# lab-incert/peba1

Hardware: AMD Instinct MI355X
Metric: bootstrapped gates/sec (blind rotations/s) over the PEBA1 match path, and end-to-end match ms (higher is better)
Workload: dtype u32

## Files before the change

### __graft_entry__.py

```python
import os
import subprocess
import sys
import tempfile

ROOT = os.path.dirname(os.path.abspath(__file__))
if ROOT not in sys.path:
    sys.path.insert(0, ROOT)


def build():
    from peba1_amd.kernel_id import kernels_sha16
    mix_path = os.path.join(ROOT, "profiles", "isa_mix.json")
    sha, stale = kernels_sha16(), True
    if os.path.exists(mix_path):
        import json
        with open(mix_path) as f:
            stale = json.load(f).get("kernels_sha16") != sha
    env = dict(os.environ)
    asm = os.path.join(tempfile.gettempdir(), f"peba1_kernels_{sha}.s")
    if stale:
        env["EMIT_KERNEL_ASM"] = asm
    subprocess.check_call(["bash", os.path.join(ROOT, "peba1_amd", "csrc", "build.sh")], env=env)
    if stale:
        try:
            subprocess.check_call([sys.executable, os.path.join(ROOT, "tools", "isa_mix.py"), asm, "--json", mix_path, "--sha", sha],
                                  stdout=subprocess.DEVNULL)
        except (subprocess.CalledProcessError, OSError) as e:
            print(f"__graft_entry__.build: tools/isa_mix.py could not summarise the kernel listing ({e}); "
                  f"profiles/isa_mix.json left as it was", file=sys.stderr)
        if os.path.exists(asm):
            os.remove(asm)
    subprocess.check_call(["make", "-s", "-C", os.path.join(ROOT, "oracle")])
    if os.path.exists("/root/reference/src/Math.cpp"):
        subprocess.check_call(["make", "-s", "-C", os.path.join(ROOT, "oracle"), "ref"])
    import peba1_amd
    from peba1_amd import lib, circuits, dist
    lib.load()
    circuits.load()
    dist.load()


def smoke():
    import numpy as np
    from oracle import pyoracle as O
    from peba1_amd import api, lib

    L = lib.load()
    seed = 0x5EBA2
    pp = api.ParameterSet(128)
    ks = api.SecretKeySet(pp, seed, device=True)
    oks = O.KeySet(O.params("P128"), seed)
    L.tfhe_hip_set_encrypt_seed(1)
    a = api.CiphertextArray(pp, 4).encrypt([0, 0, 1, 1], ks)
    b = api.CiphertextArray(pp, 4).encrypt([0, 1, 0, 1], ks)
# ... 19 lines not shown
```

### include/tfhe_hip.h

```cpp
#ifndef TFHE_HIP_H
#define TFHE_HIP_H

#include <stdio.h>

#include "tfhe/tfhe_core.h"

#ifdef __cplusplus
extern "C" {
#endif

enum TfheHipGate {
    TFHE_HIP_NAND = 0, TFHE_HIP_OR, TFHE_HIP_AND, TFHE_HIP_NOR, TFHE_HIP_XOR, TFHE_HIP_XNOR,
    TFHE_HIP_ANDNY, TFHE_HIP_ANDYN, TFHE_HIP_ORNY, TFHE_HIP_ORYN
};

const char *tfhe_hip_last_error(void);
void tfhe_hip_clear_error(void);

int tfhe_hip_set_device(int device);
int tfhe_hip_get_device(void);
int tfhe_hip_device_pci_bus_id(char *out, int len);

TFheGateBootstrappingParameterSet *tfhe_hip_new_parameters(
    int32_t n, int32_t N, int32_t k, int32_t l, int32_t Bgbit, int32_t ks_t, int32_t ks_basebit,
// ... 150 lines not shown

int tfhe_hip_test_stage_place(int64_t pos, int64_t capacity, int32_t outstanding, int64_t bytes, int64_t *out4);

void tfhe_hip_test_set_alloc_cap(int64_t bytes);

int tfhe_hip_test_schedule(const int32_t *ops5, int32_t count, int32_t unit, int32_t balance, int32_t *levels_out);
int tfhe_hip_test_level_plan(const int32_t *ops5, const int32_t *op_keys, int32_t count, int32_t nkeys, int32_t unit,
                             int32_t balance, int32_t *levels_out, int32_t *sizes6, int32_t *rot_off, int32_t *ks_off,
                             int32_t *rot_koff, int32_t *ks_koff, int32_t *rot_key, int32_t *rots6, int32_t *kss4);
int tfhe_hip_test_level_plan3(const int32_t *ops5, const int32_t *op_keys, int32_t count, int32_t nkeys, int32_t unit,
                              int32_t balance, int32_t *levels_out, int32_t *sizes6, int32_t *rot_off, int32_t *ks_off,
                              int32_t *rot_koff, int32_t *ks_koff, int32_t *rot_key, int32_t *rots8, int32_t *kss4);
int tfhe_hip_test_level_plan_lut(const int32_t *ops10, const int32_t *op_keys, int32_t count, int32_t nkeys, int32_t unit,
                                 int32_t balance, int32_t reuse, int32_t *levels_out, int32_t *shared_with, int32_t *sizes6,
                                 int32_t *rot_off, int32_t *ks_off, int32_t *rot_koff, int32_t *ks_koff, int32_t *rot_key,
                                 int32_t *rots9, int32_t *kss4);
int tfhe_hip_test_level_plan_multi(const int32_t *ops16, const int32_t *op_keys, int32_t count, int32_t nkeys, int32_t unit,
                                   int32_t balance, int32_t reuse, const int32_t *dead_slots, int32_t ndead,
                                   int32_t *levels_out, int32_t *shared_with, int32_t *sizes6, int32_t *rot_off, int32_t *ks_off,
                                   int32_t *rot_koff, int32_t *ks_koff, int32_t *rot_key, int32_t *rots10, int32_t *kss4);
int tfhe_hip_test_level_plan_lin(const int32_t *ops16, const int32_t *op_keys, int32_t count, int32_t nkeys, int32_t unit,
                                 int32_t balance, int32_t reuse, const int32_t *dead_slots, int32_t ndead,
                                 const int32_t *lin_terms2, int32_t nterms, int32_t *levels_out, int32_t *ranks_out,
                                 int32_t *shared_with, int32_t *sizes6, int32_t *rot_off, int32_t *ks_off, int32_t *rot_koff,
                                 int32_t *ks_koff, int32_t *rot_key, int32_t *rots10, int32_t *kss4, int32_t *lin_sizes2,
                                 int32_t *lin_level_off, int32_t *lin_launch_off, int32_t *lin_launch_rank, int32_t *lins35);
int tfhe_hip_test_level_plan_full(const int32_t *ops16, const int32_t *op_keys, int32_t count, int32_t nkeys, int32_t unit,
                                  int32_t balance, int32_t reuse, const int32_t *dead_slots, int32_t ndead,
                                  const int32_t *lin_terms2, int32_t nterms, int32_t *levels_out, int32_t *ranks_out,
                                  int32_t *shared_with, int32_t *sizes6, int32_t *rot_off, int32_t *ks_off, int32_t *rot_koff,
                                  int32_t *ks_koff, int32_t *rot_key, int32_t *rots10, int32_t *kss4, int32_t *lin_sizes2,
                                  int32_t *lin_level_off, int32_t *lin_launch_off, int32_t *lin_launch_rank, int32_t *lins35,
                                  int32_t *not_off, int32_t *nots2);
int tfhe_hip_test_br_plan(int32_t N, int32_t l, int32_t Bgbit, const int32_t *tunings4, int32_t cu_count, int32_t count,
                          int32_t flags, int32_t *out3);
int tfhe_hip_test_ks_plan(int32_t n, int32_t N, int32_t k, int32_t ks_t, int32_t ks_basebit, const int32_t *tunings5,
                          int32_t cu_count, int32_t count, int64_t *out6);
int tfhe_hip_test_ks_plan_form(int32_t n, int32_t N, int32_t k, int32_t ks_t, int32_t ks_basebit, const int32_t *tunings5,
                               int32_t cu_count, int32_t count, int64_t *out7);
int tfhe_hip_test_wg_times(const TFheGateBootstrappingCloudKeySet *bk, int32_t width, uint64_t *times4, double *launch_ms);

typedef struct TfheHipPackingKey TfheHipPackingKey;
TfheHipPackingKey *tfhe_hip_new_packing_key(const TFheGateBootstrappingSecretKeySet *secret, int32_t pk_t, int32_t pk_basebit);
TfheHipPackingKey *tfhe_hip_new_packing_key_seeded(const TFheGateBootstrappingSecretKeySet *secret, int32_t pk_t,
                                                   int32_t pk_basebit, uint64_t seed);
TfheHipPackingKey *tfhe_hip_new_packing_key_from_words(const TFheGateBootstrappingParameterSet *params, int32_t pk_t,
                                                       int32_t pk_basebit, const Torus32 *words);
void tfhe_hip_delete_packing_key(TfheHipPackingKey *key);
const Torus32 *tfhe_hip_packing_key_words(const TfheHipPackingKey *key, int64_t *count);
int tfhe_hip_packing_key_decomposition(const TfheHipPackingKey *key, int32_t *pk_t, int32_t *pk_basebit);
int tfhe_hip_pack_samples(const TfheHipPackingKey *key, const LweSample *samples, int32_t count,
                          const TFheGateBootstrappingCloudKeySet *bk, Torus32 *out_words);
int tfhe_hip_pack_samples_device(const TfheHipPackingKey *key, const LweSample *samples, int32_t count,
                                 const TFheGateBootstrappingCloudKeySet *bk, void *device_words);
int tfhe_hip_packed_phase(const TFheGateBootstrappingSecretKeySet *secret, const Torus32 *words, Torus32 *out_phases);
int tfhe_hip_packed_decrypt_bits(const TFheGateBootstrappingSecretKeySet *secret, const Torus32 *words, int32_t count,
                                 int32_t *out_bits);
int tfhe_hip_test_pack_bounds(int32_t N, int32_t rows, int32_t basebit);

int tfhe_hip_ring_encrypt(const TFheGateBootstrappingSecretKeySet *secret, const Torus32 *mu, Torus32 *out_words);
int tfhe_hip_ring_encrypt_seeded(const TFheGateBootstrappingSecretKeySet *secret, const Torus32 *mu, Torus32 *out_words,
                                 uint64_t seed);
int tfhe_hip_ring_encrypt_bits(const TFheGateBootstrappingSecretKeySet *secret, const int32_t *bits, int32_t count,
                               Torus32 *out_words);
int tfhe_hip_ring_encrypt_bits_seeded(const TFheGateBootstrappingSecretKeySet *secret, const int32_t *bits, int32_t count,
                                      Torus32 *out_words, uint64_t seed);
// ... 129 lines not shown
```

### peba1_amd/csrc/launch_plan.hpp

```cpp
#pragma once
#include <algorithm>
#include <cstddef>

#include "br_forms.hpp"

namespace tfhe_hip {

struct LaunchTunings {
    int br_variant = -1;
    int br8_max_rotations = 1 << 30;
    int br_tail8 = 1;
    int br_digit_table = 1;
    int ks_target_blocks = 32768;
    int ks_max_splits = 48;
    int ks_split_ties = 0;
    int ks_tile = 16;
    int ks_index = 1;
};

inline void fill_form_ok(bool form_ok[BR_FORM_COUNT][3], int N, int l, int Bgbit) {
    for (int f = 0; f < BR_FORM_COUNT; ++f)
        for (int t = 0; t < 3; ++t) form_ok[f][t] = br_form_admissible(f, N, l, Bgbit, t);
}

struct BrPlan { int form; int tables; int tail; };

inline BrPlan plan_br(const bool form_ok[BR_FORM_COUNT][3], int N, int l, const LaunchTunings &t, int cu_count, int count,
                      bool stamps, bool acc_dump) {
    int form;
    if (t.br_variant == 4 && N == 1024) form = BR_FORM_WAVE2;
    else if (t.br_variant == 2 || N == 2048) form = BR_FORM_SPLIT;
    else if (t.br8_max_rotations > 0 && count <= std::min(t.br8_max_rotations, cu_count) && l >= 2 && !stamps)
        form = BR_FORM_WAVE8;
    else form = BR_FORM_WIDE4;
    if (stamps && N == 1024) form = BR_FORM_WIDE4;
// ... 34 lines not shown
                       (threads == 128 || threads == 192 || threads == 320);
    if (!tiled) return KsPlan{KS_FORM_PERGATE, 0};
    return KsPlan{t.ks_index ? KS_FORM_INDEX : KS_FORM_STRIP, tile};
}

inline bool ks_tiled(const LaunchTunings &t, int count, const KsShape &p) { return plan_ks(t, count, p).form != KS_FORM_PERGATE; }

inline int ks_splits(const LaunchTunings &t, int cu_count, int cnt, const KsShape &p) {
    int splits = 1;
    const KsPlan plan = plan_ks(t, cnt, p);
    if (plan.form != KS_FORM_PERGATE) {
        const int tile = plan.tile;
        const int threads = ks_threads(p);
        int per_cu = std::max(1, (tile == 16 ? 16 : tile == 24 ? 12 : 8) / (threads / 64));
        if (plan.form == KS_FORM_STRIP) {
            const size_t lds = (size_t)16 * threads * 16 + (size_t)tile * 65 * 4;
            per_cu = std::max(1, std::min((int)((160 * 1024) / lds), 8 / (threads / 64)));
        }
        const long long slots = (long long)cu_count * per_cu;
        const long long tiles = (cnt + tile - 1) / tile;
        const int lo = std::max(2, (p.nin + 63) / 64);
        double best = -1.0;
        for (int sp = lo; sp <= t.ks_max_splits; ++sp) {
            const long long blocks = tiles * sp, rounds = (blocks + slots - 1) / slots;
            const double eff = (double)blocks / (double)(rounds * slots);
            if (t.ks_split_ties ? eff >= best - 1e-9 : eff > best + 1e-9) { best = eff; splits = sp; }
        }
    } else {
        while (splits < t.ks_max_splits && cnt * splits * 2 <= t.ks_target_blocks) splits *= 2;
    }
    return splits;
}

inline size_t ks_partial_bytes(const LaunchTunings &t, int cu_count, int count, const KsShape &p) {
    size_t most = 0;
    const int chunk = ks_tiled(t, count, p) ? KS_CHUNK : count;
    for (int done = 0; done < count; done += chunk) {
        const int cnt = std::min(chunk, count - done), splits = ks_splits(t, cu_count, cnt, p);
        if (splits > 1) most = std::max(most, (size_t)cnt * splits * p.ct_stride * 4);
    }
    return most;
}

}
```

### peba1_amd/csrc/recorder.cpp

```cpp
#include "recorder.hpp"

#include <algorithm>
#include <cstdio>
#include <cstdlib>
#include <cstring>
#include <utility>
#include <vector>

#include "op_graph.hpp"

namespace tfhe_hip {
namespace {

const uint8_t GATE_TT[10][4] = {
    {1, 1, 1, 0}, {0, 1, 1, 1}, {0, 0, 0, 1}, {1, 0, 0, 0}, {0, 1, 1, 0}, {1, 0, 0, 1},
    {0, 1, 0, 0}, {0, 0, 1, 0}, {1, 1, 0, 1}, {1, 0, 1, 1},
};

struct Recorder {
    std::recursive_mutex mtx;
    bool deferred = true;
    std::vector<const TFheGateBootstrappingCloudKeySet *> keys;
    uint16_t cur_key = 0;
    SlotPool *pool = nullptr;
    bool batch_keys = false;
    OpGraph<SlotPool> graph;
    bool balance_levels = true;
    std::vector<PendingOp> flight_ops;
    std::vector<LinTerm> flight_terms;
    SlotPool *flight_pool = nullptr;
    std::vector<const TFheGateBootstrappingCloudKeySet *> flight_keys;
    bool eliminate_dead = true;
    bool fold_constants = false;
};
Recorder &rec() {
    static Recorder r;
    static bool init = [] {
        if (const char *e = std::getenv("TFHE_HIP_DEFERRED")) r.deferred = std::atoi(e) != 0;
        if (const char *e = std::getenv("TFHE_HIP_FOLD_CONSTANTS")) r.fold_constants = std::atoi(e) != 0;
        if (const char *e = std::getenv("TFHE_HIP_BATCH_KEYS")) r.batch_keys = std::atoi(e) != 0;
        return true;
    }();
    (void)init;
    return r;
}

void release_refs(SlotPool *pool, const PendingOp &op, const LinTerm *terms) {
    for_each_src(op, terms, [&](int32_t s) { pool->release(s); });
    for_each_dst(op, [&](int32_t d) { pool->release(d); });
}

bool same_evaluation_params(const Params &a, const Params &b) {
    return a.n == b.n && a.N == b.N && a.k == b.k && a.l == b.l && a.Bgbit == b.Bgbit && a.ks_t == b.ks_t &&
           a.ks_basebit == b.ks_basebit;
}

void select_key(const TFheGateBootstrappingCloudKeySet *bk) {
    Recorder &r = rec();
    auto known = std::find(r.keys.begin(), r.keys.end(), bk);
    if (known == r.keys.end() && !r.graph.ops().empty()) {
        if (!r.batch_keys || pool_of_key(bk) != r.pool || !same_evaluation_params(bk->bk->p, r.keys.front()->bk->p))
            flush_locked();
    }
    if (r.graph.ops().empty()) r.keys.clear();
    known = std::find(r.keys.begin(), r.keys.end(), bk);
    if (known == r.keys.end()) {
        if (r.keys.size() > UINT16_MAX) flush_locked();
        if (r.graph.ops().empty()) r.keys.clear();
        r.keys.push_back(bk);
        known = r.keys.end() - 1;
    }
    r.cur_key = (uint16_t)(known - r.keys.begin());
}
// ... 253 lines not shown
        std::memset(result->a, 0, (size_t)bk->params->in_out_params->n * sizeof(Torus32));
        result->b = value ? (1 << 29) : -(1 << 29);
    }
}

void record_copy_locked(LweSample *result, const LweSample *ca, const TFheGateBootstrappingCloudKeySet *bk) {
    Recorder &r = rec();
    begin_op(bk);
    if (result == ca) return;
    bind_pool(result, r.pool);
    const int32_t s = ensure_slot(ca, r.pool);
    r.pool->retain(s);
    repoint(result, r.pool, s);
    if (!r.deferred) sync_sample_locked(result);
}

void finish_flight_locked() {
    Recorder &r = rec();
    Engine::get().wait_flight();
    for (const PendingOp &op : r.flight_ops) release_refs(r.flight_pool, op, r.flight_terms.data());
    r.flight_ops.clear();
    r.flight_terms.clear();
    r.flight_pool = nullptr;
    r.flight_keys.clear();
}

int flush_locked(bool wait) {
    Recorder &r = rec();
    if (!r.graph.ops().empty() && r.eliminate_dead) Engine::get().stats.dead_gates += r.graph.eliminate_dead(*r.pool);
    if (r.graph.ops().empty()) { if (wait) finish_flight_locked(); return 0; }
    SlotPool *pool = r.pool;
    const std::vector<PendingOp> &ops = r.graph.ops();
    std::vector<int32_t> lvl, alap;
    const int levels = schedule_levels(ops, r.graph.max_level(), r.balance_levels, Engine::get().cu_count(), lvl, &alap, r.graph.terms());
    if (const char *trace = std::getenv("TFHE_HIP_TRACE_DAG")) {
        if (FILE *f = std::fopen(trace, "w")) {
            for (size_t i = 0; i < ops.size(); ++i)
                std::fprintf(f, "%d %d %d %d %d %d %d %d\n", (int)ops[i].kind, ops[i].level, alap[i], lvl[i],
                             ops[i].dst, ops[i].a, ops[i].b, ops[i].c);
            std::fclose(f);
        }
    }
    std::vector<int32_t> remap(r.keys.size(), -1);
    for (const PendingOp &op : ops) remap[op.key] = 0;
    std::vector<const TFheGateBootstrappingCloudKeySet *> used;
    std::vector<const DeviceKeyImage *> images;
    for (size_t k = 0; k < r.keys.size(); ++k)
        if (remap[k] == 0) { remap[k] = (int32_t)used.size(); used.push_back(r.keys[k]); images.push_back(r.keys[k]->bk->dev); }
    LevelPlan plan;
    if (used.size() == r.keys.size()) {
        plan = build_level_plan(ops, lvl, levels, (int)used.size(), r.graph.terms());
    } else {
        std::vector<PendingOp> rekeyed = ops;
        for (PendingOp &op : rekeyed) op.key = (uint16_t)remap[op.key];
        plan = build_level_plan(rekeyed, lvl, levels, (int)used.size(), r.graph.terms());
    }
    finish_flight_locked();
    Engine::get().execute(images, pool, std::move(plan), wait);
    for (const PendingOp &op : ops) {
        for_each_dst(op, [&](int32_t d) {
            pool->level[d] = 0;
            pool->pending[d] = 0;
        });
        if (wait) release_refs(pool, op, r.graph.terms());
    }
    if (!wait) { r.flight_pool = pool; r.flight_keys = std::move(used); }
    r.graph.clear(wait ? nullptr : &r.flight_ops, wait ? nullptr : &r.flight_terms);
    return levels;
}

void flush_pending_locked(bool wait) { if (!rec().graph.ops().empty()) flush_locked(wait); }

void forget_key_locked(const TFheGateBootstrappingCloudKeySet *bk) {
    Recorder &r = rec();
    const bool pending = std::find(r.keys.begin(), r.keys.end(), bk) != r.keys.end();
    const bool flying = std::find(r.flight_keys.begin(), r.flight_keys.end(), bk) != r.flight_keys.end();
    if (pending || flying) { flush_locked(); r.keys.clear(); }
}

bool deferred_mode() { return rec().deferred; }

bool set_deferred_locked(bool on) { return std::exchange(rec().deferred, on); }

bool set_batch_keys_locked(bool on) { return std::exchange(rec().batch_keys, on); }

bool set_recorder_tuning_locked(const char *name, bool on) {
    Recorder &r = rec();
    bool *knob = std::strcmp(name, "reuse_gates") == 0      ? &r.graph.reuse
                 : std::strcmp(name, "eliminate_dead") == 0 ? &r.eliminate_dead
                 : std::strcmp(name, "fold_constants") == 0 ? &r.fold_constants
                 : std::strcmp(name, "balance_levels") == 0 ? &r.balance_levels
                 : std::strcmp(name, "batch_keys") == 0     ? &r.batch_keys
                                                            : nullptr;
    if (knob) *knob = on;
    return knob != nullptr;
}

}
```

### peba1_amd/csrc/recorder.hpp

```cpp
#pragma once
#include <cstdint>
#include <mutex>

#include "engine.hpp"
#include "../../include/tfhe/tfhe.h"

namespace tfhe_hip {
#pragma GCC visibility push(hidden)

constexpr int32_t SLOT_HOST = -1;
constexpr int32_t SLOT_ZERO = -2;

void bind_pool(const LweSample *sample, SlotPool *pool);
SlotPool *pool_of_sample(const LweSample *sample);

std::unique_lock<std::recursive_mutex> recorder_lock();
SlotPool *pool_of_key(const TFheGateBootstrappingCloudKeySet *bk);

void record_gate2_locked(int code, LweSample *result, const LweSample *a, const LweSample *b,
                         const TFheGateBootstrappingCloudKeySet *bk);
void record_not_locked(LweSample *result, const LweSample *a, const TFheGateBootstrappingCloudKeySet *bk);
void record_mux_locked(LweSample *result, const LweSample *a, const LweSample *b, const LweSample *c,
                       const TFheGateBootstrappingCloudKeySet *bk);
void record_gate3_locked(int gate, int negate_mask, LweSample *result, const LweSample *a, const LweSample *b,
                         const LweSample *c, const TFheGateBootstrappingCloudKeySet *bk);
void record_lut_locked(int32_t lut, LweSample *result, int nin, const LweSample *const *in, const int32_t *coef, int32_t c0,
                       const TFheGateBootstrappingCloudKeySet *bk);
void record_lutm_locked(int32_t lut, int32_t spec, int nout, LweSample *const *result, int nin, const LweSample *const *in,
                        const int32_t *coef, int32_t c0, const TFheGateBootstrappingCloudKeySet *bk);
void record_linear_locked(LweSample *result, int nin, const LweSample *const *in, const int32_t *coef, int32_t c0,
                          const TFheGateBootstrappingCloudKeySet *bk);
void forget_lutm_locked(int32_t lut, int32_t spec);
void forget_lut_locked(int32_t lut);
void record_constant_locked(LweSample *result, int32_t value, const TFheGateBootstrappingCloudKeySet *bk);
void record_copy_locked(LweSample *result, const LweSample *a, const TFheGateBootstrappingCloudKeySet *bk);

int32_t alloc_slot(SlotPool *pool);
int32_t ensure_slot(const LweSample *s, SlotPool *pool);
void repoint(LweSample *s, SlotPool *pool, int32_t slot);
void sync_sample_locked(const LweSample *s);

int flush_locked(bool wait = true);
void flush_pending_locked(bool wait = true);
void finish_flight_locked();
void forget_key_locked(const TFheGateBootstrappingCloudKeySet *bk);
bool deferred_mode();
bool set_deferred_locked(bool on);
bool set_batch_keys_locked(bool on);
bool set_recorder_tuning_locked(const char *name, bool on);
#pragma GCC visibility pop

}
```

### peba1_amd/csrc/scheduler.cpp

```cpp
#include "scheduler.hpp"

#include "engine.hpp"

#include <algorithm>
#include <queue>
#include <unordered_map>

namespace tfhe_hip {

namespace {
struct HeapItem {
    int32_t alap, idx;
    bool operator>(const HeapItem &o) const { return alap != o.alap ? alap > o.alap : idx > o.idx; }
};
}


int schedule_levels(const std::vector<PendingOp> &ops, int asap_depth, bool balance, int unit,
                    std::vector<int32_t> &lvl, std::vector<int32_t> *alap_out, const LinTerm *terms) {
    const int n = (int)ops.size();
    lvl.resize(n);
    for (int i = 0; i < n; ++i) lvl[i] = ops[i].level;
    if (alap_out) *alap_out = lvl;
    if (!balance || asap_depth <= 2 || n < 4 * unit) return asap_depth;

    int32_t max_slot = -1;
    for (int i = 0; i < n; ++i) for_each_dst(ops[i], [&](int32_t d) { max_slot = std::max(max_slot, d); });
    std::vector<int32_t> producer((size_t)max_slot + 1, -1);
    for (int i = 0; i < n; ++i)
        for_each_dst(ops[i], [&](int32_t d) { if (producer[d] < 0) producer[d] = i; });

    std::vector<size_t> pred_at(n);
    size_t pred_room = 0;
    for (int i = 0; i < n; ++i) { pred_at[i] = pred_room; pred_room += 3 + (size_t)op_terms(ops[i]); }
    std::vector<int32_t> pred(pred_room, -1), npred(n, 0), succ_off(n + 1, 0);
    for (int i = 0; i < n; ++i) {
        for_each_src(ops[i], terms, [&](int32_t src) {
            const int32_t pr = src <= max_slot ? producer[src] : -1;
            if (pr < 0 || pr >= i) return;
            bool dup = false;
            for (int t = 0; t < npred[i]; ++t) dup |= pred[pred_at[i] + t] == pr;
            if (dup) return;
            pred[pred_at[i] + npred[i]++] = pr;
            ++succ_off[pr + 1];
        });
    }
    for (int i = 0; i < n; ++i) succ_off[i + 1] += succ_off[i];
    std::vector<int32_t> succ(succ_off[n]), cursor(succ_off.begin(), succ_off.end() - 1);
    for (int i = 0; i < n; ++i)
        for (int t = 0; t < npred[i]; ++t) succ[cursor[pred[pred_at[i] + t]]++] = i;

    std::vector<int32_t> alap(n, asap_depth);
// ... 42 lines not shown
    std::vector<int32_t> batch;
    std::vector<long long> due(asap_depth + 2, 0);
    for (int i = 0; i < n; ++i) due[alap[i]] += op_rotations(ops[i]);
    for (int L = 1; L <= asap_depth; ++L) {
        for (int32_t i : avail[L]) heap.push(HeapItem{alap[i], i});
        const long long levels_left = asap_depth - L + 1;
        const long long base = remaining <= (long long)unit * levels_left ? unit : 2LL * unit;
        long long cap = base, running = 0, excess = 0;
        const int horizon = std::min(asap_depth, L + 1023);
        for (int D = L; D <= horizon; ++D) {
            running += due[D];
            excess = std::max(excess, running - base * (long long)(D - L + 1));
        }
        while (excess > cap - base && cap < 16LL * unit) cap *= 2;
        long long width = 0;
        batch.clear();
        auto take = [&](long long limit, bool forced_only) {
            while (!heap.empty()) {
                const HeapItem top = heap.top();
                const int w = op_rotations(ops[top.idx]);
                if (top.alap > L && (forced_only || width + w > limit)) break;
                heap.pop();
                lvl[top.idx] = L;
                width += w;
                due[top.alap] -= w;
                batch.push_back(top.idx);
            }
        };
        take(cap, false);
        if (width > cap) take((width + 2LL * unit - 1) / (2LL * unit) * (2LL * unit), false);
        remaining -= width;
        for (int32_t i : batch) release_successors(i, L, release_successors);
    }
    return asap_depth;
}

static void plan_linear_ops(LevelPlan &plan, const std::vector<PendingOp> &ops, const std::vector<int32_t> &lvl, int levels,
                            const LinTerm *terms) {
    int32_t max_slot = -1;
    size_t nlin = 0;
    for (const PendingOp &op : ops)
        if (op.kind == OP_LIN) { max_slot = std::max(max_slot, op.dst); ++nlin; }
    if (!nlin) return;
    std::vector<int32_t> producer((size_t)max_slot + 1, -1);
    plan.op_rank.assign(ops.size(), 0);
    std::vector<std::pair<int64_t, int32_t>> order;
    order.reserve(nlin);
    for (size_t i = 0; i < ops.size(); ++i) {
        const PendingOp &op = ops[i];
        if (op.kind != OP_LIN) continue;
        int32_t rank = 0;
        for (int t = 0; t < op.nout; ++t) {
            const int32_t s = terms[op.spec + t].slot;
            const int32_t pr = s <= max_slot ? producer[(size_t)s] : -1;
            if (pr >= 0 && lvl[(size_t)pr] == lvl[i]) rank = std::max(rank, plan.op_rank[(size_t)pr] + 1);
        }
        plan.op_rank[i] = rank;
        producer[(size_t)op.dst] = (int32_t)i;
        order.emplace_back((int64_t)lvl[i] << 32 | (uint32_t)rank, (int32_t)i);
    }
    std::stable_sort(order.begin(), order.end(), [](const auto &x, const auto &y) { return x.first < y.first; });
    plan.lins.resize(nlin);
    plan.lin_level_off.assign((size_t)levels + 2, 0);
    plan.lin_launch_off.assign(1, 0);
    for (size_t j = 0; j < nlin; ++j) {
        const PendingOp &op = ops[(size_t)order[j].second];
// ... 103 lines not shown
```

### peba1_amd/csrc/scheduler.hpp

```cpp
#pragma once
#include <cstddef>
#include <cstdint>
#include <utility>
#include <vector>

namespace tfhe_hip {

struct PendingOp {
    uint8_t kind;
    int32_t dst, a, b, c;
    int32_t level;
    uint16_t key = 0;
    int32_t lut = -1;
    int32_t sa = 0, sb = 0, sc = 0, c0 = 0;
    int32_t spec = -1;
    int32_t nout = 0;
    int32_t dsts[4] = {-1, -1, -1, -1};
};
constexpr uint8_t OP_MUX = 16, OP_NOT = 17;
constexpr uint8_t OP_LUT = 64;
constexpr uint8_t OP_GATE3 = 32, OP_GATE3_END = OP_GATE3 + 3 * 8;
inline bool op_is_gate3(int kind) { return kind >= OP_GATE3 && kind < OP_GATE3_END; }
inline bool op_kind_valid(int kind) { return (kind >= 0 && kind < 10) || kind == OP_MUX || kind == OP_NOT || op_is_gate3(kind); }
inline bool op_kind_valid_lut(int kind) { return op_kind_valid(kind) || kind == OP_LUT; }
// ... 40 lines not shown
    const int32_t s = GATE3_LIN[(kind - OP_GATE3) >> 3];
    return ((kind - OP_GATE3) >> operand) & 1 ? -s : s;
}

struct OpKey {
    int32_t kind, a, b, c, key;
    int32_t lut, sa, sb, sc, c0;
    int32_t spec = -1;
    bool operator==(const OpKey &o) const {
        return kind == o.kind && a == o.a && b == o.b && c == o.c && key == o.key && lut == o.lut && sa == o.sa &&
               sb == o.sb && sc == o.sc && c0 == o.c0 && spec == o.spec;
    }
};
struct OpKeyHash {
    size_t operator()(const OpKey &k) const {
        uint64_t h = ((uint64_t)(uint32_t)k.a << 32 | (uint32_t)k.b) * 0x9E3779B97F4A7C15ull;
        h ^= ((uint64_t)(uint32_t)k.c << 8 | (uint32_t)k.kind) * 0xC2B2AE3D27D4EB4Full;
        h ^= (uint64_t)(uint32_t)k.key * 0x165667B19E3779F9ull;
        if (k.kind == OP_LUT || k.kind == OP_LUTM) {
            h ^= ((uint64_t)(uint32_t)k.lut << 32 | (uint32_t)k.c0) * 0xD6E8FEB86659FD93ull;
            h ^= (uint64_t)(uint32_t)(k.spec + 1) * 0x9FB21C651E98DF25ull;
            h ^= ((uint64_t)(uint32_t)k.sa << 40 ^ (uint64_t)(uint32_t)k.sb << 20 ^ (uint32_t)k.sc) * 0xFF51AFD7ED558CCDull;
        }
        return (size_t)(h ^ (h >> 29));
    }
};
inline OpKey op_key(const PendingOp &op) {
    int32_t a = op.a, b = op.b;
    if (op.kind < OP_MUX && GATE_LIN[op.kind].sa == GATE_LIN[op.kind].sb && b < a) std::swap(a, b);
    if (op.kind != OP_LUT && op.kind != OP_LUTM) return OpKey{op.kind, a, b, op.c, op.key, -1, 0, 0, 0, 0};
    return OpKey{op.kind, a, b, op.c, op.key, op.lut, op.sa, op.sb, op.sc, op.c0, op.kind == OP_LUTM ? op.spec : -1};
}

int schedule_levels(const std::vector<PendingOp> &ops, int asap_depth, bool balance, int unit,
                    std::vector<int32_t> &lvl, std::vector<int32_t> *alap_out = nullptr, const LinTerm *terms = nullptr);

struct LevelPlan;
__attribute__((visibility("hidden"))) LevelPlan build_level_plan(const std::vector<PendingOp> &ops,
                                                                 const std::vector<int32_t> &lvl, int levels, int nkeys = 1,
                                                                 const LinTerm *terms = nullptr);

}
```

### peba1_amd/csrc/shim.cpp

```cpp
#include <cstddef>
#include <cstdio>
#include <cstdlib>
#include <cstring>
#include <algorithm>
#include <numeric>
#include <string>
#include <vector>

#include "br_forms.hpp"
#include "engine.hpp"
#include "op_graph.hpp"
#include "recorder.hpp"
#include "scheduler.hpp"
#include "../../include/tfhe/tfhe.h"

using namespace tfhe_hip;

namespace tfhe_hip {
const std::string &last_error_ref();
bool io_forget_owned_cloud(const void *ks);
bool io_forget_owned_secret(const void *ks);
TFheGateBootstrappingCloudKeySet *io_adopt_cloud(TfheHipCloudKey *ck);
}

// ... 934 lines not shown
int tfhe_hip_set_batch_keys(int on) {
    auto g = recorder_lock();
    return set_batch_keys_locked(on != 0) ? 1 : 0;
}

static int test_build_ops(const int32_t *ops5, int32_t count, std::vector<PendingOp> &ops) {
    for (int32_t i = 0; i < count; ++i)
        if (!op_kind_valid(ops5[5 * (size_t)i])) { set_error("test schedule: unknown op kind"); return -1; }
    ops.resize((size_t)count);
    std::vector<int32_t> slot_level;
    int depth = 0;
    auto level_of = [&](int32_t s) { return s >= 0 && (size_t)s < slot_level.size() ? slot_level[s] : 0; };
    for (int32_t i = 0; i < count; ++i) {
        const int32_t *o = ops5 + 5 * (size_t)i;
        PendingOp op{(uint8_t)o[0], o[1], o[2], o[3], o[4], 0};
        const int32_t in = std::max(level_of(op.a), std::max(level_of(op.b), level_of(op.c)));
        op.level = op.kind == OP_NOT ? in : in + 1;
        if ((size_t)op.dst >= slot_level.size()) slot_level.resize((size_t)op.dst + 1, 0);
        slot_level[op.dst] = op.level;
        depth = std::max(depth, op.level);
        ops[i] = op;
    }
    return depth;
}

int tfhe_hip_test_schedule(const int32_t *ops5, int32_t count, int32_t unit, int32_t balance, int32_t *levels_out) {
    std::vector<PendingOp> ops;
    const int depth = test_build_ops(ops5, count, ops);
    if (depth < 0) return -1;
    std::vector<int32_t> lvl;
    const int d = schedule_levels(ops, depth, balance != 0, unit, lvl);
    for (int32_t i = 0; i < count; ++i) levels_out[i] = lvl[i];
    return d;
}

struct TestLinPlan {
    const int32_t *terms2; int32_t nterms;
    int32_t *ranks_out, *sizes2, *level_off, *launch_off, *launch_rank, *descs35;
    int32_t *not_off = nullptr, *nots2 = nullptr;
};
static int test_level_plan(const int32_t *ops5, const int32_t *op_keys, int32_t count, int32_t nkeys, int32_t unit,
                           int32_t balance, int32_t *levels_out, int32_t *sizes6, int32_t *rot_off, int32_t *ks_off,
                           int32_t *rot_koff, int32_t *ks_koff, int32_t *rot_key, int32_t *rots, int rot_words, int32_t *kss4,
                           bool lut_ops = false, int32_t reuse = 0, int32_t *shared_with = nullptr, int rec_words = 10,
                           const int32_t *dead_slots = nullptr, int32_t ndead = 0, const TestLinPlan *lin = nullptr) {
    if (count < 0 || nkeys < 1 || nkeys > UINT16_MAX) { set_error("test_level_plan: bad count or nkeys"); return -1; }
    for (int32_t i = 0; i < count; ++i)
        if (op_keys[i] < 0 || op_keys[i] >= nkeys) { set_error("test_level_plan: key index out of range"); return -1; }
    std::vector<PendingOp> ops;
    std::vector<int32_t> op_of_record;
    std::vector<LinTerm> terms;
    int depth;
    if (!lut_ops) {
        depth = test_build_ops(ops5, count, ops);
        if (depth < 0) return -1;
        for (int32_t i = 0; i < count; ++i) ops[i].key = (uint16_t)op_keys[i];
    } else {
        struct SlotTable {
            std::vector<int32_t> ref, level;
            std::vector<uint8_t> pending;
            void retain(int32_t s) { ++ref[(size_t)s]; }
            void release(int32_t s) { --ref[(size_t)s]; }
            int32_t refs(int32_t s) const { return ref[(size_t)s]; }
        };
        const int id_words = rec_words == 16 ? 4 : 0;
        int32_t top = 0;
// ... 299 lines not shown
```

### peba1_amd/lib.py

```python
import ctypes as C
import os

_HERE = os.path.dirname(os.path.abspath(__file__))
LIB_PATH = os.environ.get("PEBA1_TFHE_HIP_LIB") or os.path.join(_HERE, "libtfhe-hip.so")
CIRCUITS_PATH = os.path.join(_HERE, "libpeba1-circuits.so")


class LweSample(C.Structure):
    _fields_ = [("a", C.POINTER(C.c_int32)), ("b", C.c_int32), ("slot", C.c_int32),
                ("current_variance", C.c_double)]


class LweParams(C.Structure):
    _fields_ = [("n", C.c_int32), ("alpha_min", C.c_double), ("alpha_max", C.c_double)]


class TLweParams(C.Structure):
    _fields_ = [("N", C.c_int32), ("k", C.c_int32), ("alpha_min", C.c_double), ("alpha_max", C.c_double)]


class TGswParams(C.Structure):
    _fields_ = [("l", C.c_int32), ("Bgbit", C.c_int32), ("Bg", C.c_int32), ("halfBg", C.c_int32),
                ("maskMod", C.c_uint32), ("tlwe_params", C.POINTER(TLweParams)), ("kpl", C.c_int32),
                ("offset", C.c_uint32)]
# ... 138 lines not shown
    "tfhe_hip_lut_bootstrap_batch": (C.c_int, [C.c_void_p, LS, C.c_int32, C.POINTER(LS), I32P, C.c_int32, C.c_int32, CK]),
    "tfhe_hip_new_lut_multi": (C.c_void_p, [C.c_void_p, C.c_int32, I32P, I32P, I32P, I32P]),
    "tfhe_hip_new_lut_multi_from_tables": (C.c_void_p, [PS, C.c_int32, C.c_int32, C.c_int32, I32P]),
    "tfhe_hip_delete_lut_multi": (None, [C.c_void_p]),
    "tfhe_hip_lut_multi_nout": (C.c_int32, [C.c_void_p]),
    "tfhe_hip_lut_multi_output": (C.c_int32, [C.c_void_p, C.c_int32, I32P, I32P, I32P]),
    "tfhe_hip_lut_multi_words": (I32P, [C.c_void_p, I32P]),
    "tfhe_hip_lut_bootstrap_multi": (None, [C.c_void_p, C.POINTER(LS), C.c_int32, C.POINTER(LS), I32P, C.c_int32, CK]),
    "tfhe_hip_lut_bootstrap_multi_batch": (C.c_int, [C.c_void_p, C.POINTER(LS), C.c_int32, C.POINTER(LS), I32P, C.c_int32,
                                                     C.c_int32, CK]),
    "tfhe_hip_linear": (None, [LS, C.c_int32, C.POINTER(LS), I32P, C.c_int32, CK]),
    "tfhe_hip_linear_batch": (C.c_int, [LS, C.c_int32, C.POINTER(LS), I32P, C.c_int32, C.c_int32, CK]),
    "tfhe_hip_sym_encrypt_torus": (None, [LS, C.c_int32, SK]),
    "tfhe_hip_sym_phase": (C.c_int32, [LS, SK]),
    "tfhe_hip_set_tuning": (C.c_int, [C.c_char_p, C.c_int64]),
    "tfhe_hip_test_form_admissible": (C.c_int, [C.c_int, C.c_int32, C.c_int32, C.c_int32, C.c_int]),
    "tfhe_hip_test_set_alloc_cap": (None, [C.c_int64]),
    "tfhe_hip_test_stage_place": (C.c_int, [C.c_int64, C.c_int64, C.c_int32, C.c_int64, C.POINTER(C.c_int64)]),
    "tfhe_hip_get_stats": (None, [C.POINTER(StatsWhole)]),
    "tfhe_hip_reset_stats": (None, []),
    "tfhe_hip_set_kernel_timing": (None, [C.c_int]),
    "tfhe_hip_last_flush_keys": (C.c_int, []),
    "tfhe_hip_set_batch_keys": (C.c_int, [C.c_int]),
    "tfhe_hip_test_schedule": (C.c_int, [I32P, C.c_int32, C.c_int32, C.c_int32, I32P]),
    "tfhe_hip_test_level_plan": (C.c_int, [I32P, I32P, C.c_int32, C.c_int32, C.c_int32, C.c_int32] + [I32P] * 9),
    "tfhe_hip_test_level_plan3": (C.c_int, [I32P, I32P, C.c_int32, C.c_int32, C.c_int32, C.c_int32] + [I32P] * 9),
    "tfhe_hip_test_level_plan_lut": (C.c_int, [I32P, I32P, C.c_int32, C.c_int32, C.c_int32, C.c_int32, C.c_int32] + [I32P] * 10),
    "tfhe_hip_test_level_plan_multi": (C.c_int, [I32P, I32P, C.c_int32, C.c_int32, C.c_int32, C.c_int32, C.c_int32, I32P,
                                                 C.c_int32] + [I32P] * 10),
    "tfhe_hip_test_level_plan_lin": (C.c_int, [I32P, I32P, C.c_int32, C.c_int32, C.c_int32, C.c_int32, C.c_int32, I32P,
                                               C.c_int32, I32P, C.c_int32] + [I32P] * 16),
    "tfhe_hip_test_level_plan_full": (C.c_int, [I32P, I32P, C.c_int32, C.c_int32, C.c_int32, C.c_int32, C.c_int32, I32P,
                                                C.c_int32, I32P, C.c_int32] + [I32P] * 18),
    "tfhe_hip_test_br_plan": (C.c_int, [C.c_int32] * 3 + [I32P, C.c_int32, C.c_int32, C.c_int32, I32P]),
    "tfhe_hip_test_ks_plan": (C.c_int, [C.c_int32] * 5 + [I32P, C.c_int32, C.c_int32, C.POINTER(C.c_int64)]),
    "tfhe_hip_test_ks_plan_form": (C.c_int, [C.c_int32] * 5 + [I32P, C.c_int32, C.c_int32, C.POINTER(C.c_int64)]),
    "tfhe_hip_kernel_negacyclic":(C.c_int, [CK, I32P, I32P, I32P, C.c_int32]),
    "tfhe_hip_kernel_bootstrap_woks": (C.c_int, [CK, I32P, C.c_int32, I32P, I32P]),
    "tfhe_hip_kernel_lut_bootstrap_woks": (C.c_int, [CK, I32P, C.c_int32, I32P, I32P, C.c_int32, I32P, I32P]),
    "tfhe_hip_kernel_lut_bootstrap_multi_woks": (C.c_int, [CK, I32P, C.c_int32, I32P, I32P, C.c_int32, I32P, I32P, C.c_int32,
                                                           I32P, I32P]),
    "tfhe_hip_kernel_keyswitch": (C.c_int, [CK, I32P, C.c_int32, I32P]),
    "tfhe_hip_new_packing_key": (C.c_void_p, [SK, C.c_int32, C.c_int32]),
    "tfhe_hip_new_packing_key_seeded": (C.c_void_p, [SK, C.c_int32, C.c_int32, C.c_uint64]),
    "tfhe_hip_new_packing_key_from_words": (C.c_void_p, [PS, C.c_int32, C.c_int32, I32P]),
    "tfhe_hip_delete_packing_key": (None, [C.c_void_p]),
    "tfhe_hip_packing_key_words": (I32P, [C.c_void_p, C.POINTER(C.c_int64)]),
    "tfhe_hip_packing_key_decomposition": (C.c_int, [C.c_void_p, I32P, I32P]),
    "tfhe_hip_pack_samples": (C.c_int, [C.c_void_p, LS, C.c_int32, CK, I32P]),
    "tfhe_hip_pack_samples_device": (C.c_int, [C.c_void_p, LS, C.c_int32, CK, C.c_void_p]),
    "tfhe_hip_packed_phase": (C.c_int, [SK, I32P, I32P]),
    "tfhe_hip_packed_decrypt_bits": (C.c_int, [SK, I32P, C.c_int32, I32P]),
    "tfhe_hip_test_pack_bounds": (C.c_int, [C.c_int32, C.c_int32, C.c_int32]),
    "tfhe_hip_kernel_pack": (C.c_int, [C.c_void_p, CK, I32P, C.c_int32, C.c_int32, I32P]),
    "tfhe_hip_ring_encrypt": (C.c_int, [SK, I32P, I32P]),
    "tfhe_hip_ring_encrypt_seeded": (C.c_int, [SK, I32P, I32P, C.c_uint64]),
    "tfhe_hip_ring_encrypt_bits": (C.c_int, [SK, I32P, C.c_int32, I32P]),
    "tfhe_hip_ring_encrypt_bits_seeded": (C.c_int, [SK, I32P, C.c_int32, I32P, C.c_uint64]),
    "tfhe_hip_unpack_samples": (C.c_int, [CK, I32P, C.c_int32, I32P, C.c_int32, LS]),
    "tfhe_hip_unpack_samples_scattered": (C.c_int, [CK, I32P, C.c_int32, I32P, C.c_int32, C.POINTER(LS)]),
    "tfhe_hip_unpack_samples_device": (C.c_int, [CK, C.c_void_p, C.c_int32, I32P, C.c_int32, LS]),
    "tfhe_hip_kernel_ring_extract": (C.c_int, [CK, I32P, C.c_int32, I32P, C.c_int32, I32P]),
    "tfhe_hip_new_compressed_cloud_key": (C.c_void_p, [SK]),
    "tfhe_hip_new_compressed_cloud_key_seeded": (C.c_void_p, [SK, C.c_uint64, U32P]),
    "tfhe_hip_new_compressed_cloud_key_from_words": (C.c_void_p, [PS, U32P, I32P, I32P]),
    "tfhe_hip_delete_compressed_cloud_key": (None, [C.c_void_p]),
# ... 80 lines not shown
```

Measured before the change: 108,900.

## Relevel gates across DAG slack using a measured per-level cost table

```diff
diff --git a/__graft_entry__.py b/__graft_entry__.py
--- a/__graft_entry__.py
+++ b/__graft_entry__.py
@@ -20,6 +20,7 @@
     asm = os.path.join(tempfile.gettempdir(), f"peba1_kernels_{sha}.s")
     if stale:
         env["EMIT_KERNEL_ASM"] = asm
+    subprocess.check_call([sys.executable, os.path.join(ROOT, "tools", "level_cost_inc.py")])
     subprocess.check_call(["bash", os.path.join(ROOT, "peba1_amd", "csrc", "build.sh")], env=env)
     if stale:
         try:
diff --git a/include/tfhe_hip.h b/include/tfhe_hip.h
--- a/include/tfhe_hip.h
+++ b/include/tfhe_hip.h
@@ -206,6 +206,13 @@
                                   int32_t *ks_koff, int32_t *rot_key, int32_t *rots10, int32_t *kss4, int32_t *lin_sizes2,
                                   int32_t *lin_level_off, int32_t *lin_launch_off, int32_t *lin_launch_rank, int32_t *lins35,
                                   int32_t *not_off, int32_t *nots2);
+int tfhe_hip_test_level_slack(const int32_t *ops5, int32_t count, int32_t unit, int32_t level_slack, const int32_t *cost_widths,
+                              const double *cost_us, int32_t ncost, int32_t period, int32_t *levels_out, int32_t *widths_out,
+                              double *cost_out2);
+int tfhe_hip_test_level_cost(int32_t n, int32_t N, int32_t k, int32_t l, int32_t Bgbit, int32_t ks_t, int32_t ks_basebit,
+                             int32_t cu_count, int32_t width, double *us_out);
+int tfhe_hip_test_set_level_cost(const int32_t *cost_widths, const double *cost_us, int32_t ncost);
+int tfhe_hip_last_level_slack(double *out4);
 int tfhe_hip_test_br_plan(int32_t N, int32_t l, int32_t Bgbit, const int32_t *tunings4, int32_t cu_count, int32_t count,
                           int32_t flags, int32_t *out3);
 int tfhe_hip_test_ks_plan(int32_t n, int32_t N, int32_t k, int32_t ks_t, int32_t ks_basebit, const int32_t *tunings5,
diff --git a/peba1_amd/csrc/launch_plan.hpp b/peba1_amd/csrc/launch_plan.hpp
--- a/peba1_amd/csrc/launch_plan.hpp
+++ b/peba1_amd/csrc/launch_plan.hpp
@@ -1,6 +1,8 @@
 #pragma once
 #include <algorithm>
+#include <climits>
 #include <cstddef>
+#include <cstdint>
 
 #include "br_forms.hpp"
 
@@ -101,6 +103,82 @@
     return splits;
 }
 
+struct LevelCost {
+    const int32_t *width = nullptr;
+    const double *us = nullptr;
+    int n = 0;
+    int period = 0;
+};
+
+inline long long level_cost_fold(const LevelCost &c, long long width) {
+    const long long top = c.width[c.n - 1];
+    if (width <= top || c.period <= 0 || c.period > top - c.width[0]) return 0;
+    return (width - top + c.period - 1) / c.period;
+}
+
+inline double level_cost_at(const LevelCost &c, long long width) {
+    if (width <= 0 || c.n <= 0) return 0.0;
+    if (width <= c.width[0] || c.n == 1) return c.us[0];
+    const long long top = c.width[c.n - 1], fold = level_cost_fold(c, width);
+    if (fold > 0) return level_cost_at(c, width - fold * c.period) + (double)fold * (c.us[c.n - 1] - level_cost_at(c, top - c.period));
+    const int32_t *hi = std::lower_bound(c.width, c.width + c.n, (int32_t)std::min<long long>(width, top));
+    const int j = (int)(hi - c.width);
+    return c.us[j - 1] + (c.us[j] - c.us[j - 1]) * (double)(width - c.width[j - 1]) / (double)(c.width[j] - c.width[j - 1]);
+}
+
+inline int level_cost_steps(const LevelCost &c, long long width, int dir, long long *out, int most) {
+    if (c.n <= 0) return 0;
+    const long long shift = level_cost_fold(c, width) * c.period, at = width - shift;
+    int count = 0;
+    if (dir < 0) {
+        for (int j = (int)(std::lower_bound(c.width, c.width + c.n, (int32_t)std::min<long long>(at, INT32_MAX)) - c.width) - 1;
+             j >= 0 && count < most; --j)
+            out[count++] = c.width[j] + shift;
+    } else {
+        for (int j = (int)(std::upper_bound(c.width, c.width + c.n, (int32_t)std::min<long long>(at, INT32_MAX)) - c.width);
+             j < c.n && count < most; ++j)
+            out[count++] = c.width[j] + shift;
+    }
+    return count;
+}
+
+struct LevelCostEntry {
+    int n, N, k, l, Bgbit, ks_t, ks_basebit;
+    int cus;
+    int br_variant, br8_max_rotations, br_tail8, br_digit_table, ks_tile, ks_index, ks_max_splits, ks_target_blocks,
+        ks_split_ties;
+    int count;
+    const int32_t *width;
+    const double *us;
+};
+#if __has_include("level_cost_tables.inc")
+#include "level_cost_tables.inc"
+#else
+#warning "level_cost_tables.inc is missing (run tools/level_cost_inc.py before peba1_amd/csrc/build.sh): this library knows no level-cost table and the tuning level_slack does nothing"
+static constexpr LevelCostEntry LEVEL_COST_TABLES[1] = {};
+static constexpr int LEVEL_COST_TABLE_COUNT = 0;
+#endif
+
+struct LevelCostSet { int n, N, k, l, Bgbit, ks_t, ks_basebit; };
+
+inline LevelCost level_cost_table(const LevelCostSet &p, int cus, const LaunchTunings &t) {
+    for (int i = 0; i < LEVEL_COST_TABLE_COUNT; ++i) {
+        const LevelCostEntry &e = LEVEL_COST_TABLES[i];
+        if (e.n == p.n && e.N == p.N && e.k == p.k && e.l == p.l && e.Bgbit == p.Bgbit && e.ks_t == p.ks_t &&
+            e.ks_basebit == p.ks_basebit && e.cus == cus && e.br_variant == t.br_variant &&
+            e.br8_max_rotations == t.br8_max_rotations && e.br_tail8 == t.br_tail8 && e.br_digit_table == t.br_digit_table &&
+            e.ks_tile == t.ks_tile && e.ks_index == t.ks_index && e.ks_max_splits == t.ks_max_splits &&
+            e.ks_target_blocks == t.ks_target_blocks && e.ks_split_ties == t.ks_split_ties)
+            return LevelCost{e.width, e.us, e.count, 2 * e.cus};
+    }
+    return LevelCost{};
+}
+
+inline double level_cost_us(int width, const LevelCostSet &p, int cus, const LaunchTunings &t) {
+    const LevelCost c = level_cost_table(p, cus, t);
+    return c.n ? level_cost_at(c, width) : -1.0;
+}
+
 inline size_t ks_partial_bytes(const LaunchTunings &t, int cu_count, int count, const KsShape &p) {
     size_t most = 0;
     const int chunk = ks_tiled(t, count, p) ? KS_CHUNK : count;
diff --git a/peba1_amd/csrc/recorder.cpp b/peba1_amd/csrc/recorder.cpp
--- a/peba1_amd/csrc/recorder.cpp
+++ b/peba1_amd/csrc/recorder.cpp
@@ -26,6 +26,10 @@
     bool batch_keys = false;
     OpGraph<SlotPool> graph;
     bool balance_levels = true;
+    bool level_slack = true;
+    std::vector<int32_t> cost_width;
+    std::vector<double> cost_us;
+    LevelSlackReport last_slack;
     std::vector<PendingOp> flight_ops;
     std::vector<LinTerm> flight_terms;
     SlotPool *flight_pool = nullptr;
@@ -39,6 +43,7 @@
         if (const char *e = std::getenv("TFHE_HIP_DEFERRED")) r.deferred = std::atoi(e) != 0;
         if (const char *e = std::getenv("TFHE_HIP_FOLD_CONSTANTS")) r.fold_constants = std::atoi(e) != 0;
         if (const char *e = std::getenv("TFHE_HIP_BATCH_KEYS")) r.batch_keys = std::atoi(e) != 0;
+        if (const char *e = std::getenv("TFHE_HIP_LEVEL_SLACK")) r.level_slack = std::atoi(e) != 0;
         return true;
     }();
     (void)init;
@@ -358,7 +363,17 @@
     SlotPool *pool = r.pool;
     const std::vector<PendingOp> &ops = r.graph.ops();
     std::vector<int32_t> lvl, alap;
-    const int levels = schedule_levels(ops, r.graph.max_level(), r.balance_levels, Engine::get().cu_count(), lvl, &alap, r.graph.terms());
+    LevelCost cost;
+    if (r.level_slack && !r.cost_width.empty()) {
+        cost = LevelCost{r.cost_width.data(), r.cost_us.data(), (int)r.cost_width.size(), 0};
+    } else if (r.level_slack) {
+        const DevParams &dp = r.keys[ops[0].key]->bk->dev->dp;
+        cost = level_cost_table(LevelCostSet{dp.n, dp.N, dp.k, dp.l, dp.Bgbit, dp.ks_t, dp.ks_basebit}, Engine::get().cu_count(),
+                                Engine::get().tunings);
+    }
+    const int levels = schedule_levels(ops, r.graph.max_level(), r.balance_levels, Engine::get().cu_count(), lvl, &alap, r.graph.terms(),
+                                       &cost, &r.last_slack);
+    r.last_slack.pool_slots = (long long)pool->in_use();
     if (const char *trace = std::getenv("TFHE_HIP_TRACE_DAG")) {
         if (FILE *f = std::fopen(trace, "w")) {
             for (size_t i = 0; i < ops.size(); ++i)
@@ -410,9 +425,21 @@
 
 bool set_batch_keys_locked(bool on) { return std::exchange(rec().batch_keys, on); }
 
+void set_level_cost_locked(const int32_t *widths, const double *us, int count) {
+    Recorder &r = rec();
+    r.cost_width.assign(widths, widths + count);
+    r.cost_us.assign(us, us + count);
+}
+
+void last_level_slack_locked(double *out4) {
+    const LevelSlackReport &s = rec().last_slack;
+    out4[0] = s.us_before; out4[1] = s.us_after; out4[2] = (double)s.moved; out4[3] = (double)s.pool_slots;
+}
+
 bool set_recorder_tuning_locked(const char *name, bool on) {
     Recorder &r = rec();
     bool *knob = std::strcmp(name, "reuse_gates") == 0      ? &r.graph.reuse
+                 : std::strcmp(name, "level_slack") == 0    ? &r.level_slack
                  : std::strcmp(name, "eliminate_dead") == 0 ? &r.eliminate_dead
                  : std::strcmp(name, "fold_constants") == 0 ? &r.fold_constants
                  : std::strcmp(name, "balance_levels") == 0 ? &r.balance_levels
diff --git a/peba1_amd/csrc/recorder.hpp b/peba1_amd/csrc/recorder.hpp
--- a/peba1_amd/csrc/recorder.hpp
+++ b/peba1_amd/csrc/recorder.hpp
@@ -47,6 +47,8 @@
 bool deferred_mode();
 bool set_deferred_locked(bool on);
 bool set_batch_keys_locked(bool on);
+void set_level_cost_locked(const int32_t *widths, const double *us, int count);
+void last_level_slack_locked(double *out4);
 bool set_recorder_tuning_locked(const char *name, bool on);
 #pragma GCC visibility pop
 
diff --git a/peba1_amd/csrc/scheduler.cpp b/peba1_amd/csrc/scheduler.cpp
--- a/peba1_amd/csrc/scheduler.cpp
+++ b/peba1_amd/csrc/scheduler.cpp
@@ -1,6 +1,7 @@
 #include "scheduler.hpp"
 
 #include "engine.hpp"
+#include "launch_plan.hpp"
 
 #include <algorithm>
 #include <queue>
@@ -13,11 +14,100 @@
     int32_t alap, idx;
     bool operator>(const HeapItem &o) const { return alap != o.alap ? alap > o.alap : idx > o.idx; }
 };
+
+struct SuccLists { const std::vector<int32_t> &off, &to; };
+struct PredLists { const std::vector<size_t> &at; const std::vector<int32_t> &of, &count; };
+void relevel_by_cost(const std::vector<PendingOp> &ops, int depth, const LevelCost &cost, const SuccLists &succ,
+                     const PredLists &pred, std::vector<int32_t> &lvl, LevelSlackReport *report) {
+    const int n = (int)ops.size();
+    std::vector<long long> width((size_t)depth + 2, 0);
+    std::vector<std::vector<int32_t>> at((size_t)depth + 2);
+    for (int i = 0; i < n; ++i) {
+        if (op_is_linear(ops[i].kind)) continue;
+        width[(size_t)lvl[i]] += op_rotations(ops[i]);
+        at[(size_t)lvl[i]].push_back(i);
+    }
+    auto total = [&] { double t = 0; for (int L = 1; L <= depth; ++L) t += level_cost_at(cost, width[(size_t)L]); return t; };
+    const double before = total();
+    if (report) { report->us_before = report->us_after = before; report->moved = 0; }
+    const std::vector<int32_t> kept = lvl;
+    auto latest = [&](int32_t i, auto &&self) -> int32_t {
+        int32_t ub = depth;
+        for (int32_t e = succ.off[i]; e < succ.off[i + 1] && ub > lvl[i]; ++e) {
+            const int32_t s = succ.to[e];
+            ub = std::min(ub, op_is_linear(ops[s].kind) ? self(s, self) : lvl[s] - 1);
+        }
+        return ub;
+    };
+    std::vector<HeapItem> movable;
+    long long moved_gates = 0;
+    constexpr int STEPS = 16, AHEAD = 4;
+    for (int L = 1; L < depth; ++L) {
+        movable.clear();
+        long long free_rot = 0;
+        for (int32_t i : at[(size_t)L]) {
+            const int32_t ub = latest(i, latest);
+            if (ub > L) { movable.push_back(HeapItem{-ub, i}); free_rot += op_rotations(ops[i]); }
+        }
+        if (!free_rot) continue;
+        std::sort(movable.begin(), movable.end(), [](const HeapItem &x, const HeapItem &y) { return y > x; });
+        const long long w = width[(size_t)L];
+        double best_gain = 0;
+        long long best_m = 0;
+        int best_j = 0;
+        size_t reach = movable.size();
+        for (int j = 1; j <= AHEAD && L + j <= depth; ++j) {
+            while (reach > 0 && -movable[reach - 1].alap < L + j) free_rot -= op_rotations(ops[movable[--reach].idx]);
+            if (!free_rot) break;
+            const long long nx = width[(size_t)(L + j)];
+            const double now = level_cost_at(cost, w) + level_cost_at(cost, nx);
+            auto consider = [&](long long m) {
+                if (m <= 0 || m > free_rot) return;
+                const double gain = now - level_cost_at(cost, w - m) - level_cost_at(cost, nx + m);
+                if (gain <= 0.005 * now) return;
+                if (gain > best_gain + 1e-9 || (gain > best_gain - 1e-9 && j == best_j && m < best_m)) { best_gain = gain; best_m = m; best_j = j; }
+            };
+            long long steps[STEPS];
+            consider(free_rot);
+            for (int k = level_cost_steps(cost, w, -1, steps, STEPS); k-- > 0;) consider(w - steps[k]);
+            for (int k = level_cost_steps(cost, nx, +1, steps, STEPS); k-- > 0;) consider(steps[k] - nx);
+        }
+        if (!best_m) continue;
+        const int to = L + best_j;
+        long long m = 0;
+        size_t take = 0;
+        for (; take < movable.size() && -movable[take].alap >= to; ++take) {
+            const int r = op_rotations(ops[movable[take].idx]);
+            if (m + r > best_m) break;
+            m += r;
+        }
+        const double now = level_cost_at(cost, w) + level_cost_at(cost, width[(size_t)to]);
+        if (now - level_cost_at(cost, w - m) - level_cost_at(cost, width[(size_t)to] + m) <= 0.005 * now) continue;
+        for (size_t t = 0; t < take; ++t) {
+            lvl[movable[t].idx] = to;
+            at[(size_t)to].push_back(movable[t].idx);
+        }
+        width[(size_t)L] -= m;
+        width[(size_t)to] += m;
+        moved_gates += (long long)take;
+    }
+    const double after = total();
+    if (!moved_gates || !(after < before)) { lvl = kept; return; }
+    for (int i = 0; i < n; ++i) {
+        if (!op_is_linear(ops[i].kind)) continue;
+        int32_t l = 0;
+        for (int t = 0; t < pred.count[i]; ++t) l = std::max(l, lvl[pred.of[pred.at[i] + t]]);
+        lvl[i] = l;
+    }
+    if (report) { report->us_after = after; report->moved = moved_gates; }
+}
 }
 
 
 int schedule_levels(const std::vector<PendingOp> &ops, int asap_depth, bool balance, int unit,
-                    std::vector<int32_t> &lvl, std::vector<int32_t> *alap_out, const LinTerm *terms) {
+                    std::vector<int32_t> &lvl, std::vector<int32_t> *alap_out, const LinTerm *terms,
+                    const LevelCost *cost, LevelSlackReport *report) {
+    if (report) *report = LevelSlackReport{};
     const int n = (int)ops.size();
     lvl.resize(n);
     for (int i = 0; i < n; ++i) lvl[i] = ops[i].level;
@@ -126,6 +216,7 @@
         remaining -= width;
         for (int32_t i : batch) release_successors(i, L, release_successors);
     }
+    if (cost && cost->n > 0) relevel_by_cost(ops, asap_depth, *cost, SuccLists{succ_off, succ}, PredLists{pred_at, pred, npred}, lvl, report);
     return asap_depth;
 }
 
diff --git a/peba1_amd/csrc/scheduler.hpp b/peba1_amd/csrc/scheduler.hpp
--- a/peba1_amd/csrc/scheduler.hpp
+++ b/peba1_amd/csrc/scheduler.hpp
@@ -96,8 +96,11 @@
     return OpKey{op.kind, a, b, op.c, op.key, op.lut, op.sa, op.sb, op.sc, op.c0, op.kind == OP_LUTM ? op.spec : -1};
 }
 
+struct LevelCost;
+struct LevelSlackReport { double us_before = 0, us_after = 0; long long moved = 0, pool_slots = 0; };
 int schedule_levels(const std::vector<PendingOp> &ops, int asap_depth, bool balance, int unit,
-                    std::vector<int32_t> &lvl, std::vector<int32_t> *alap_out = nullptr, const LinTerm *terms = nullptr);
+                    std::vector<int32_t> &lvl, std::vector<int32_t> *alap_out = nullptr, const LinTerm *terms = nullptr,
+                    const LevelCost *cost = nullptr, LevelSlackReport *report = nullptr);
 
 struct LevelPlan;
 __attribute__((visibility("hidden"))) LevelPlan build_level_plan(const std::vector<PendingOp> &ops,
diff --git a/peba1_amd/csrc/shim.cpp b/peba1_amd/csrc/shim.cpp
--- a/peba1_amd/csrc/shim.cpp
+++ b/peba1_amd/csrc/shim.cpp
@@ -990,6 +990,63 @@
     const int d = schedule_levels(ops, depth, balance != 0, unit, lvl);
     for (int32_t i = 0; i < count; ++i) levels_out[i] = lvl[i];
     return d;
+}
+
+int tfhe_hip_test_level_slack(const int32_t *ops5, int32_t count, int32_t unit, int32_t level_slack, const int32_t *cost_widths,
+                              const double *cost_us, int32_t ncost, int32_t period, int32_t *levels_out, int32_t *widths_out,
+                              double *cost_out2) {
+    if (!ops5 || count < 0 || unit < 1 || ncost < 0 || period < 0 || (ncost > 0 && (!cost_widths || !cost_us)) || !levels_out || !widths_out ||
+        !cost_out2) {
+        set_error("test_level_slack: bad arguments");
+        return -1;
+    }
+    for (int32_t j = 0; j < ncost; ++j)
+        if (cost_widths[j] < 1 || (j > 0 && cost_widths[j] <= cost_widths[j - 1]) || !(cost_us[j] >= 0)) {
+            set_error("test_level_slack: the table's widths must ascend from 1 on, its costs must not be negative");
+            return -1;
+        }
+    std::vector<PendingOp> ops;
+    const int depth = test_build_ops(ops5, count, ops);
+    if (depth < 0) return -1;
+    std::vector<int32_t> lvl;
+    const LevelCost table{cost_widths, cost_us, ncost, period}, none;
+    LevelSlackReport report;
+    schedule_levels(ops, depth, true, unit, lvl, nullptr, nullptr, level_slack ? &table : &none, &report);
+    std::fill(widths_out, widths_out + depth + 1, 0);
+    for (int32_t i = 0; i < count; ++i) {
+        levels_out[i] = lvl[i];
+        widths_out[lvl[i]] += op_rotations(ops[i]);
+    }
+    cost_out2[0] = cost_out2[1] = 0;
+    for (int L = 1; L <= depth; ++L) cost_out2[0] += level_cost_at(table, widths_out[L]);
+    cost_out2[1] = report.moved ? report.us_before : cost_out2[0];
+    return depth;
+}
+
+int tfhe_hip_test_level_cost(int32_t n, int32_t N, int32_t k, int32_t l, int32_t Bgbit, int32_t ks_t, int32_t ks_basebit,
+                             int32_t cu_count, int32_t width, double *us_out) {
+    if (!us_out) { set_error("test_level_cost: null output"); return -1; }
+    *us_out = level_cost_us(width, LevelCostSet{n, N, k, l, Bgbit, ks_t, ks_basebit}, cu_count, LaunchTunings{});
+    return 0;
+}
+
+int tfhe_hip_test_set_level_cost(const int32_t *cost_widths, const double *cost_us, int32_t ncost) {
+    if (ncost < 0 || (ncost > 0 && (!cost_widths || !cost_us))) { set_error("test_set_level_cost: bad arguments"); return -1; }
+    for (int32_t j = 0; j < ncost; ++j)
+        if (cost_widths[j] < 1 || (j > 0 && cost_widths[j] <= cost_widths[j - 1]) || !(cost_us[j] >= 0)) {
+            set_error("test_set_level_cost: the table's widths must ascend from 1 on, its costs must not be negative");
+            return -1;
+        }
+    auto g = recorder_lock();
+    set_level_cost_locked(cost_widths, cost_us, ncost);
+    return 0;
+}
+
+int tfhe_hip_last_level_slack(double *out4) {
+    if (!out4) { set_error("last_level_slack: null output"); return -1; }
+    auto g = recorder_lock();
+    last_level_slack_locked(out4);
+    return 0;
 }
 
 struct TestLinPlan {
diff --git a/peba1_amd/lib.py b/peba1_amd/lib.py
--- a/peba1_amd/lib.py
+++ b/peba1_amd/lib.py
@@ -194,6 +194,11 @@
                                                C.c_int32, I32P, C.c_int32] + [I32P] * 16),
     "tfhe_hip_test_level_plan_full": (C.c_int, [I32P, I32P, C.c_int32, C.c_int32, C.c_int32, C.c_int32, C.c_int32, I32P,
                                                 C.c_int32, I32P, C.c_int32] + [I32P] * 18),
+    "tfhe_hip_test_level_slack": (C.c_int, [I32P, C.c_int32, C.c_int32, C.c_int32, I32P, C.POINTER(C.c_double), C.c_int32, C.c_int32, I32P,
+                                            I32P, C.POINTER(C.c_double)]),
+    "tfhe_hip_test_level_cost": (C.c_int, [C.c_int32] * 9 + [C.POINTER(C.c_double)]),
+    "tfhe_hip_test_set_level_cost": (C.c_int, [I32P, C.POINTER(C.c_double), C.c_int32]),
+    "tfhe_hip_last_level_slack": (C.c_int, [C.POINTER(C.c_double)]),
     "tfhe_hip_test_br_plan": (C.c_int, [C.c_int32] * 3 + [I32P, C.c_int32, C.c_int32, C.c_int32, I32P]),
     "tfhe_hip_test_ks_plan": (C.c_int, [C.c_int32] * 5 + [I32P, C.c_int32, C.c_int32, C.POINTER(C.c_int64)]),
     "tfhe_hip_test_ks_plan_form": (C.c_int, [C.c_int32] * 5 + [I32P, C.c_int32, C.c_int32, C.POINTER(C.c_int64)]),
```

After: 110,300, median of 6. 1.2% higher.
